# uwoseis/zephyr

Hardware: AMD Instinct MI355X
Metric: wavefields/sec (freq x source solves/s) on 1024^2 grid (higher is better)
Workload: dtype f64

## Files before the change

include/helm.h:

```cpp
#ifndef HELM_H
#define HELM_H

#include <stddef.h>

#ifdef __cplusplus
extern "C" {
#endif

typedef struct helm_op helm_op;

enum { HELM_MINIZEPHYR = 0, HELM_EURUS = 1, HELM_3D = 2  };

enum {
    HELM_BICGSTAB = 0,
    HELM_CGNR = 1,
    HELM_AUTO = 2,
    HELM_MG = 3,
    HELM_DIRECT = 4
};

enum {
    HELM_OK = 0,
    HELM_ERR_ARG = -1,
    HELM_ERR_DEVICE = -2,
// ... 140 lines not shown
    int    auto_direct;
    int    auto_mg3;
    int    prof_ext;
    int    ws_slots;
    int    pf_prio;
    int    mg3_keep;
    int    mg3_keep_levels;
    int    mg3_galerkin;
    int    mg3_depth_model;
    int    mg3_bt_f32;
    int    mg3_otf;
    int    mg3_f32;
    double mg3_omega;
    double sync_spin_ms;
    int    sync_sleep_us;
} helm_tuning;
int helm_get_tuning(helm_tuning *out);
int helm_set_tuning(const helm_tuning *t);

int helm_direct_plan(int nz, int nx, int leaf, int *out, int cap);
int helm_direct_plan_front(int nz, int nx, int leaf, int node, long long *cells, int cap);
int helm_debug_zgemm(int device, int M, int N, int K, const double *alpha, const double *A, const double *B,
                     const double *beta, double *C, int batch);
int helm_debug_inverse(int device, int n, double *A, int batch);
int helm_debug_zgemm_bench(int device, int M, int N, int K, int batch, int variant, int reps, double *ms_out);
#define HELM_ZG_TABLE 1
#define HELM_ZG_MASKS 2
#define HELM_ZG_TM64  4
int helm_debug_zgemm_choice(int M, int N, int K, int batch, int nf_div, int force_tile, int force_slab, int have_handle, int mode, int report[5]);
typedef struct helm_zgemm_ex {
// ... 42 lines not shown
```

zephyr_amd/_lib.py:

```python
import ctypes
import os
import numpy as np

_HERE = os.path.dirname(os.path.abspath(__file__))
LIB_PATH = os.path.join(_HERE, 'libhelm.so')

HELM_MINIZEPHYR, HELM_EURUS, HELM_3D = 0, 1, 2
HELM_BICGSTAB, HELM_CGNR, HELM_AUTO, HELM_MG, HELM_DIRECT = 0, 1, 2, 3, 4
HELM_RHS_NODE_MAJOR, HELM_OUT_NODE_MAJOR, HELM_NODE_MAJOR = 1, 2, 3
METHODS = {'bicgstab': HELM_BICGSTAB, 'cgnr': HELM_CGNR, 'auto': HELM_AUTO, 'mg': HELM_MG, 'direct': HELM_DIRECT}

ERRORS = {-1: 'HELM_ERR_ARG', -2: 'HELM_ERR_DEVICE', -3: 'HELM_ERR_STATE', -4: 'HELM_ERR_UNSUPPORTED', -5: 'HELM_ERR_PML'}


class HelmError(RuntimeError):
    def __init__(self, code, text):
        self.code = code
        RuntimeError.__init__(self, '%s: %s' % (ERRORS.get(code, code), text))


class SolveOpts(ctypes.Structure):
    _fields_ = [('method', ctypes.c_int), ('rtol', ctypes.c_double), ('maxit', ctypes.c_int),
                ('check_every', ctypes.c_int), ('batch', ctypes.c_int), ('flags', ctypes.c_int)]

# ... 7 lines not shown
    _fields_ = [('solve_ms', ctypes.c_double), ('apply_ms', ctypes.c_double),
                ('apply_launches', ctypes.c_longlong), ('apply_bytes', ctypes.c_double),
                ('factor_ms', ctypes.c_double), ('gemm_ms', ctypes.c_double),
                ('gemm_launches', ctypes.c_longlong), ('gemm_flops', ctypes.c_double),
                ('gemm_big_ms', ctypes.c_double), ('gemm_big_launches', ctypes.c_longlong), ('gemm_big_flops', ctypes.c_double),
                ('gemm_bytes', ctypes.c_double), ('gemm_sol_ms', ctypes.c_double)]


class Tuning(ctypes.Structure):
    _fields_ = [('nd_leaf', ctypes.c_int), ('nd_ws_gb', ctypes.c_double), ('nd_sparse_rhs', ctypes.c_int), ('nd_stable', ctypes.c_int),
                ('nd_stable_thr', ctypes.c_double), ('nd_stable_safety', ctypes.c_double), ('nd_fused_leaf', ctypes.c_int),
                ('nd_fused_leaf_min', ctypes.c_int), ('nd_gjstep', ctypes.c_int), ('nd_gjstep_min', ctypes.c_int), ('nd_overlap', ctypes.c_int),
                ('nd_xcd_map', ctypes.c_int), ('nd_plans', ctypes.c_int), ('nd_direct_out', ctypes.c_int), ('nd_many', ctypes.c_int), ('nd_leaf_idle', ctypes.c_int), ('auto_direct', ctypes.c_int),
                ('auto_mg3', ctypes.c_int), ('prof_ext', ctypes.c_int), ('ws_slots', ctypes.c_int), ('pf_prio', ctypes.c_int),
                ('mg3_keep', ctypes.c_int), ('mg3_keep_levels', ctypes.c_int), ('mg3_galerkin', ctypes.c_int), ('mg3_depth_model', ctypes.c_int),
                ('mg3_bt_f32', ctypes.c_int), ('mg3_otf', ctypes.c_int), ('mg3_f32', ctypes.c_int), ('mg3_omega', ctypes.c_double), ('sync_spin_ms', ctypes.c_double), ('sync_sleep_us', ctypes.c_int)]


class RuntimeStats(ctypes.Structure):
    _fields_ = [('dev_allocs', ctypes.c_longlong), ('dev_alloc_bytes', ctypes.c_double), ('dev_alloc_ms', ctypes.c_double),
                ('host_allocs', ctypes.c_longlong), ('host_alloc_bytes', ctypes.c_double), ('host_alloc_ms', ctypes.c_double),
                ('events_created', ctypes.c_longlong), ('streams_created', ctypes.c_longlong),
                ('first_launches', ctypes.c_longlong), ('first_launch_ms', ctypes.c_double),
                ('kernels_registered', ctypes.c_longlong), ('kernels_resolved', ctypes.c_longlong), ('warm_ms', ctypes.c_double),
                ('dev_frees', ctypes.c_longlong), ('dev_free_ms', ctypes.c_double),
                ('sync_calls', ctypes.c_longlong), ('sync_ms', ctypes.c_double), ('slow_syncs', ctypes.c_longlong), ('worst_sync_ms', ctypes.c_double)]


class ZgemmEx(ctypes.Structure):
    _fields_ = [('device', ctypes.c_int), ('M', ctypes.c_int), ('N', ctypes.c_int), ('K', ctypes.c_int), ('batch', ctypes.c_int),
                ('lda', ctypes.c_int), ('ldb', ctypes.c_int), ('ldc', ctypes.c_int),
# ... 255 lines not shown
```

zephyr_amd/csrc/nd_factor.hip:

```cpp
#include "nd_internal.hpp"
#include <map>
#include <mutex>
#include <cstring>

namespace {

__device__ __forceinline__ long long mf_off(long long off, long long slot, int nf, int kf) { return (long long)nf * off + (long long)kf * slot; }
__device__ __forceinline__ cplx *front_entry(const NdDev &n, cplx *arenaF, cplx *fac, int r, int c, int nf = 1, int kf = 0, int fac_private = 0) {
    const int nmax = n.smax + n.mmax;
    if (r < n.smax) {
        return fac + (fac_private ? n.finv_off : mf_off(n.finv_off, (long long)n.smax * nmax, nf, kf)) + (long long)r * nmax + c;
    }
    return arenaF + mf_off(n.foff, (long long)n.mmax * nmax, nf, kf) + (long long)(r - n.smax) * nmax + c;
}

__global__ __launch_bounds__(256) void k_nd_assemble(const NdDev *nodes, int first, cplx *arenaF, cplx *fac, const cplx *planes, int nz, int nx) {
    const NdDev n = nodes[first + blockIdx.y];
    const long long N = (long long)nz * nx;
    const int tot = n.s + n.m;
    for (int a = blockIdx.x * blockDim.x + threadIdx.x; a < n.smax; a += gridDim.x * blockDim.x)
        if (a >= n.s) *front_entry(n, arenaF, fac, a, a) = cmake(1.0, 0.0);
    for (int a = blockIdx.x * blockDim.x + threadIdx.x; a < tot; a += gridDim.x * blockDim.x) {
        int z, x, ca;
        nd_cell(n, a, z, x, ca);
// ... 28 lines not shown
        map[a] = nd_pos(p, nd_local(p, nz, nx, z, x, comp));
    }
    __syncthreads();
    const cplx *Sc = arenaF + c.foff + c.smax;
    const int ldc = c.smax + c.mmax;
    for (long long e0 = (long long)blockIdx.x * chunk; e0 < total; e0 += (long long)gridDim.x * chunk) {
        const long long e1 = e0 + chunk < total ? e0 + chunk : total;
        for (long long e = e0 + threadIdx.x; e < e1; e += blockDim.x) {
            const int a = (int)(e / c.m), b2 = (int)(e - (long long)a * c.m);
            cplx *dst = front_entry(p, arenaF, fac, map[a], map[b2]);
            *dst = cadd(*dst, Sc[(long long)a * ldc + b2]);
        }
    }
}

template <bool OVR>
__global__ __launch_bounds__(256) void k_nd_build_front(const NdDev *nodes, int first, cplx *arenaF, cplx *fac, NdPlanesSet pset, int nz, int nx, int rb,
                                                        int skip22, NdDev ovr, int nf, int kfix) {
    constexpr int use_ovr = OVR ? 1 : 0;
    extern __shared__ int2 finfo[];
    const int kf = kfix >= 0 ? kfix : (int)(blockIdx.y % nf);
    const cplx *planes = pset.p[kf];
    NdDev n;
    if (OVR) n = ovr; else n = nodes[first + (kfix >= 0 ? blockIdx.y : blockIdx.y / nf)];
    const int nmax = n.smax + n.mmax;
    const int r0 = blockIdx.x * rb;
    if (r0 >= nmax) return;
    const bool h0 = n.kid[0] >= 0, h1 = n.kid[1] >= 0;
    NdDev c0 = NdDev(), c1 = NdDev();
    if (h0) c0 = nodes[n.kid[0]];
    if (h1) c1 = nodes[n.kid[1]];
// ... 34 lines not shown
            if (dz >= -1 && dz <= 1 && dx >= -1 && dx <= 1) {
                if (colmode) {
                    const int dc = ((ib.x >> 24) & 0x7f) - ca;
                    if (dc >= -1 && dc <= 1) v = planes[((long long)(dc + 1) * 9 + (dz + 1) * 3 + dx + 1) * N * n.dof + (long long)ca * N + (long long)za * nx + xa];
                } else {
                    const int blk = n.dof == 2 ? 2 * ca + ((ib.y >> 28) & 1) : 0;
                    v = planes[((long long)blk * 9 + (dz + 1) * 3 + dx + 1) * N + (long long)za * nx + xa];
                }
            }
        }
        const int b0 = (colmode ? (ib.y & 0xffff) : (ib.y & 0x3fff)) - 1, b1 = (colmode ? ((ib.y >> 16) & 0xffff) : ((ib.y >> 14) & 0x3fff)) - 1;
        if (a0 >= 0 && b0 >= 0) v = cadd(v, S0[(long long)a0 * ld0 + b0]);
        if (a1 >= 0 && b1 >= 0) v = cadd(v, S1[(long long)a1 * ld1 + b1]);
        return v;
    };
    for (int r = r0 + ty; r < r1; r += 4) {
        const int2 ia = finfo[r];
        const int cend = (skip22 && r >= n.smax) ? n.smax : nmax;
        for (int c = tx; c < cend; c += 64) *front_entry(n, arenaF, fac, r, c, nf, kf, use_ovr) = value(r, c, ia, finfo[c]);
    }
}

template <int AFTER>
__global__ __launch_bounds__(256) void k_front_cond(const cplx *M0, int ld, long long stride, const NdDev *nodes, double *out, double *rows, int smax, int nf) {
    __shared__ double red[4];
    __shared__ double dsh[LUS_NMAX];
    __shared__ unsigned char lone[LUS_NMAX];
    const cplx *M = M0 + (long long)blockIdx.x * stride;
    double *w = rows + (long long)blockIdx.x * smax;
    const int n = nodes[blockIdx.x / nf].s;
    const int lane = threadIdx.x & 63, wv = threadIdx.x >> 6;
    double best = 0.0;
    for (int i = wv; i < n; i += 4) {
        double v = 0.0, off = 0.0;
// ... 311 lines not shown
    const cplx one = cmake(1, 0), mone = cmake(-1, 0);
    for (int q = 0; q < nflag; ++q) {
        const int j = h_list[1 + q];
        NdStable S;
        S.node = g.first + j; S.group = gi; S.smax = g.smax; S.mmax = g.mmax;
        S.lu = (cplx *)helm_pool_alloc(op->device, (size_t)g.smax * nmax * sizeof(cplx));
        S.f21 = (cplx *)helm_pool_alloc(op->device, (size_t)std::max(1, g.mmax) * g.smax * sizeof(cplx));
        S.piv = (int *)helm_pool_alloc(op->device, (size_t)g.smax * sizeof(int));
        f->stable.push_back(S);
        if (!S.lu || !S.f21 || !S.piv) HELM_FAIL(op, HELM_ERR_DEVICE, "direct solver: allocation for an ill-conditioned front failed");
        NdDev n = P.nodes[S.node];
        const long long foff = (long long)nf * n.foff + (long long)kf * g.mmax * nmax;
        n.finv_off = 0; n.f12_off = g.smax;
        const int rb = std::max(std::min(nmax, 4), (nmax + 2047) / 2048);
        NdPlanesSet ps; for (int q2 = 0; q2 < ND_NF_MAX; ++q2) ps.p[q2] = planes;
        HELM_LAUNCH(k_nd_build_front<true>, dim3((nmax + rb - 1) / rb, 1), dim3(256), (size_t)nmax * sizeof(int2), st, f->pd->d_nodes, 0, arenaF, S.lu, ps, P.nz, P.nx, rb,
                           0, n, nf, kf);
        cplx *F21 = arenaF + foff, *F22 = arenaF + foff + g.smax;
        HIP_TRY(op, hipMemcpy2DAsync(S.f21, (size_t)g.smax * sizeof(cplx), F21, (size_t)nmax * sizeof(cplx), (size_t)g.smax * sizeof(cplx), (size_t)g.mmax, hipMemcpyDeviceToDevice, st));
        if (g.smax <= 64) HELM_LAUNCH(k_lu_factor64, dim3(1), dim3(256), 0, st, S.lu, nmax, g.smax, S.piv);
        else HELM_LAUNCH(k_lu_factor, dim3(1), dim3(256), 0, st, S.lu, nmax, g.smax, S.piv);
        HIP_TRY(op, hipMemcpy2DAsync(work, (size_t)g.mmax * sizeof(cplx), S.lu + g.smax, (size_t)nmax * sizeof(cplx), (size_t)g.mmax * sizeof(cplx), (size_t)g.smax, hipMemcpyDeviceToDevice, st));
        HELM_LAUNCH(k_lu_solve, dim3((g.mmax + 15) / 16), dim3(256), 0, st, (const cplx *)S.lu, nmax, g.smax, (const int *)S.piv, work, g.mmax, g.mmax);
        gemm(op, g.mmax, g.mmax, g.smax, mone, S.f21, g.smax, 0, work, g.mmax, 0, one, F22, nmax, 0, 1, nullptr);
        if (getenv("HELM_ND_DEBUG") && atoi(getenv("HELM_ND_DEBUG")) >= 3) {
            auto sum2d = [&](const void *src, size_t pitch, size_t wbytes, size_t rows_) {
                std::vector<unsigned char> h(wbytes * rows_);
                hipMemcpy2D(h.data(), wbytes, src, pitch, wbytes, rows_, hipMemcpyDeviceToHost);
                unsigned long long x = 1469598103934665603ull;
                for (unsigned char c : h) { x ^= c; x *= 1099511628211ull; }
                return x;
// ... 34 lines not shown
    if (fused_leaf && g.leaf && g.cnt >= fused_leaf_min && P.dof == 1 && P.leaf <= 8 && g.smax <= 64 && g.mmax > 0 && g.mmax <= LEAF_MP) {
        const int leaf_dbg = getenv("HELM_LEAF_DBG") ? atoi(getenv("HELM_LEAF_DBG")) : 0;
        for (int k = 0; k < nf; ++k) {
            NdFactor *f = S.f[k];
            if (f->leafflag_elems < (size_t)g.cnt) {
                if (f->d_leafflag) { hipStreamSynchronize(st); helm_pool_free(op->device, f->d_leafflag, f->leafflag_elems * sizeof(int)); f->d_leafflag = nullptr; f->leafflag_elems = 0; }
                int maxcnt = g.cnt;
                for (const NdGroup &q : P.groups) if (q.leaf) maxcnt = std::max(maxcnt, q.cnt);
                f->d_leafflag = (int *)helm_pool_alloc(op->device, (size_t)maxcnt * sizeof(int));
                if (!f->d_leafflag) HELM_FAIL(op, HELM_ERR_DEVICE, "direct solver: allocation of the leaf flags failed");
                f->leafflag_elems = (size_t)maxcnt;
            }
            for (int j0 = 0; j0 < g.cnt; j0 += 65535) {
                const int nb = std::min(65535, g.cnt - j0);
                cplx *g21b = G21 + (long long)j0 * nf * g.mmax * g.smax;
                launch_leaf_factor(st, g.smax, nb, d_nodes, g.first + j0, arenaF, f0->d_fac, g21b, S.planes[k], P.nz, P.nx, f->d_leafflag + j0, leaf_dbg, nf, k);
            }
            f->flops += (double)g.cnt * 8.0 * (2.0 * LEAF_BW * g.smax * (g.smax + g.mmax) + 3.0 * g.mmax * (g.smax + g.mmax));
        }
        return HELM_OK;
    }
    bool schur_gather = false;
    const bool packs = P.dof <= 2 ? (nmax < (1 << 14) && P.nz < 65536 && P.nx < 32768) : (nmax < 65535 && P.nz < 4096 && P.nx < 4096 && P.dof < 128);
    if ((size_t)nmax * sizeof(int2) <= 64 * 1024 && packs)
        schur_gather = !g.leaf && g.mmax > 0 && P.dof == 1;
    if ((size_t)nmax * sizeof(int2) <= 64 * 1024 && packs) {
        const int want = std::max(1, 2048 / g.cnt);
        const int rb = std::max(std::min(nmax, 4), (nmax + want - 1) / want);
        NdPlanesSet ps; for (int k = 0; k < ND_NF_MAX; ++k) ps.p[k] = S.planes[k < nf ? k : 0];
        const int chunk = 65535 / nf;
        for (int j0 = 0; j0 < g.cnt; j0 += chunk) {
            const int nb = std::min(chunk, g.cnt - j0);
            HELM_LAUNCH(k_nd_build_front<false>, dim3((nmax + rb - 1) / rb, nb * nf), dim3(256), (size_t)nmax * sizeof(int2), st, d_nodes, g.first + j0, arenaF, f0->d_fac, ps,
                               P.nz, P.nx, rb, schur_gather ? 1 : 0, NdDev(), nf, -1);
        }
    } else {
        if (nf != 1) HELM_FAIL(op, HELM_ERR_UNSUPPORTED, "direct solver: fronts of %d unknowns take the unfused build, which factors one frequency at a time", nmax);
        const cplx *planes = S.planes[0];
        if (fs > 0) HIP_TRY(op, hipMemsetAsync(F, 0, (size_t)g.cnt * fs * sizeof(cplx), st));
        HIP_TRY(op, hipMemsetAsync(Finv, 0, (size_t)g.cnt * s1 * sizeof(cplx), st));
        for (int j0 = 0; j0 < g.cnt; j0 += 65535) {
            const int nb = std::min(65535, g.cnt - j0);
            HELM_LAUNCH(k_nd_assemble, dim3((nmax + 255) / 256, nb), dim3(256), 0, st, d_nodes, g.first + j0, arenaF, f0->d_fac, planes, P.nz, P.nx);
        }
        if (!g.leaf) {
            const size_t shm = (size_t)(2 * nmax + 8) * sizeof(int);
            for (int slot = 0; slot < 2; ++slot)
                for (int j0 = 0; j0 < g.cnt; j0 += 65535) {
                    const int nb = std::min(65535, g.cnt - j0);
// ... 120 lines not shown
```

zephyr_amd/csrc/nd_gemm_body.hpp:

```cpp
#pragma once
#include "nd_internal.hpp"

static __device__ cplx g_zero_page[4];
template <int WM, int WN, int MT, int NT, int IDX, int KS, int XR = 0>
__device__ __forceinline__ void zgemm3_body(int M, int Nn, int K, cplx alpha, const cplx *A0, int lda, long long sa,
                                            const cplx *B0, int ldb, long long sb, cplx beta, cplx *C0, int ldc, long long sc, const GemmRows &R,
                                            cplx *lds) {
    static_assert(WM * WN == 4 && KS % 4 == 0, "four waves per workgroup, k groups of 4");
    static_assert(!XR || (WM == 1 && (IDX == 0 || IDX == 1)), "the extra row needs all four waves side by side and plain / row-table addressing");
    constexpr int TMM = 16 * MT * WM;
    constexpr int TM = TMM + (XR ? 1 : 0), TN = 16 * NT * WN;
    constexpr int FA = TMM / 16 + (XR ? 1 : 0), FB = TN / 16, KG = KS / 4;
    constexpr int NA = (FA * 16 * KS + 255) / 256, NB = (TN * KS + 255) / 256;
    constexpr int XP = 256 / TN;
    constexpr int ABUF = KG * FA * 64, BBUF = KG * FB * 64;
    cplx *As = lds, *Bs = lds + 2 * ABUF;
    __shared__ int kidx[IDX == 1 ? GB_KIDX : 1];
    __shared__ int4 kidx4[IDX == 2 ? GB_KIDX : 1];
    int bxi = blockIdx.x, byi = blockIdx.y, bzi = blockIdx.z;
    if (gridDim.x * gridDim.y > 1 && gridDim.z >= 16 && R.la == nullptr && !(IDX == 0 && R.ksplit > 1) && R.xcd_map && (gridDim.y == 1 || R.xcd_map > 1)) {
        const int nxt = gridDim.x, nt = gridDim.x * gridDim.y, nbz = gridDim.z;
        const int L = blockIdx.x + nxt * blockIdx.y + nt * blockIdx.z;
        const int full = (nbz / 8) * 8 * nt;
        int tile;
// ... 337 lines not shown
```

zephyr_amd/csrc/nd_internal.hpp:

```cpp
#pragma once
#include "helm_internal.hpp"
#include "direct.hpp"
#include <hip/hip_ext.h>
#include <algorithm>

struct GjPivotArgs { const cplx *T0; int ld; long long stride; int n, k0, nb; const cplx *Wc0, *Wr0; long long wstride; cplx *Pb0; long long pstride; int batch; };
struct GemmRows {
    const int4 *tabB = nullptr, *tabCi = nullptr, *tabCo = nullptr;
    int offB = 0, offCi = 0, offCo = 0, tab_stride = 0;
    const cplx *Bx = nullptr, *Cix = nullptr; cplx *Cox = nullptr;
    int ldx = 0;
    int z0 = 0;
    int fwd3 = 0;
    int zr0 = 0, zr1 = 0, zc0 = 0, zc1 = 0;
    int sk0 = 0, sk1 = 0;
    int ksplit = 0, kc = 0; long long pstride = 0;
    int dense = 0;
    const cplx *Bx2 = nullptr; int k2 = 0;
    int tm64 = 0;
    const GjPivotArgs *la = nullptr;
    int schur4 = 0;
    const NdDev *nodes = nullptr; int first = 0;
    const cplx *arenaS = nullptr;
    int nf = 1;
// ... 2 lines not shown
    const int *act_ro = nullptr;
    int idle_done = 0;
    int hint = 0;
    int ntc = 0;
    int xcd_map = 0;
    int child_rows = 0;
    int cj_out = 0; cplx oscale = {1.0, 0.0}; cplx *Cox2 = nullptr;
};
#define GB_KIDX 512

#define PNB 32
#define LEAF_BW 9
#define LEAF_MP 36
#define LUS_NMAX 128
#define ND_STABLE_CAP 32

extern thread_local hipEvent_t tl_ev0, tl_ev1;
extern thread_local int tl_nf_div;
struct NfDivScope { int prev; explicit NfDivScope(int nf) : prev(tl_nf_div) { tl_nf_div = nf < 1 ? 1 : nf; } ~NfDivScope() { tl_nf_div = prev; } };
#define ZG_LAUNCH(KERNEL, GRID, ...) do { HelmFirstLaunch fl_(HelmKernelReg<(KERNEL)>::slot); \
                                          if (tl_ev0) hipExtLaunchKernelGGL(KERNEL, GRID, dim3(256), 0, st, tl_ev0, tl_ev1, 0, __VA_ARGS__); \
                                          else hipLaunchKernelGGL(KERNEL, GRID, dim3(256), 0, st, __VA_ARGS__); } while (0)

inline double gemm_operand_bytes(int M, int Nn, int K, cplx beta, const GemmRows *rows = nullptr) {
    const bool rd = !(beta.x == 0.0 && beta.y == 0.0);
    if (rows && rows->fwd3) return 16.0 * ((double)M * K + (double)K * Nn + (double)rows->child_rows * Nn + (double)M * Nn + (double)K * Nn);
    if (rows && rows->schur4) return 16.0 * ((double)M * K + (double)K * Nn + 1.5 * (double)M * Nn);
    return 16.0 * ((double)M * K + (double)K * Nn + (double)M * Nn * (rd ? 2.0 : 1.0));
}
inline double gemm_sol_ms(double flops, double bytes) { return 1e3 * std::max(flops / 78.6e12, bytes / 8.0e12); }
// ... 105 lines not shown
    }
};

struct GemmChoice { int tile = 0, kslab = 8, xr = 0, ksplit = 0, kc = 0; };
int gemm(helm_op *op, int M, int Nn, int K, cplx alpha, const cplx *A, int lda, long long sa, const cplx *B, int ldb, long long sb,
         cplx beta, cplx *C, int ldc, long long sc, int batch, const GemmRows *rows = nullptr, GemmChoice *made = nullptr);
extern int g_gemm_tile;
extern int g_gemm_slab;
extern int g_gemm_xcd;
bool gemm_sep_bwd_small(helm_op *op, int smax, int mmax, int nrhs, const cplx *Finv, const cplx *F12, int lda, long long sa, int batch, const GemmRows &rows);
void invert(helm_op *op, cplx *M, int ld, long long stride, int n, int batch, cplx *W, long long ws, int align = 1, int base = 0);
extern int g_recurse_min;
void launch_zgemm3_la(hipStream_t st, bool latency_tile, int nb, int M, int Nn, int K, cplx alpha, const cplx *A, int lda, long long sa, const cplx *B, int ldb, long long sb,
                      cplx beta, cplx *C, int ldc, long long sc, const GemmRows &R, const GjPivotArgs &pv);
void launch_leaf_factor(hipStream_t st, int smax, int nb, const NdDev *d_nodes, int first, cplx *arenaF, cplx *fac, cplx *g21b, const cplx *planes, int nz, int nx, int *flags, int dbg,
                        int nf = 1, int kf = 0);
struct FacSet { int nf = 1; NdFactor *f[ND_NF_MAX] = {nullptr, nullptr, nullptr, nullptr}; const cplx *planes[ND_NF_MAX] = {nullptr, nullptr, nullptr, nullptr}; double rtol[ND_NF_MAX] = {0, 0, 0, 0}; };
int factor_prologue(helm_op *op, int block, NdFactor *f, const cplx *planes_in, const cplx **planes);
int factor_group(helm_op *op, NdFactor *f, size_t gi, cplx *arenaF, cplx *work, const cplx *planes);
bool merged_group(const NdPlan &P, const NdGroup &g);
void launch_lu_solve(hipStream_t st, const cplx *LU, int ld, int n, const int *piv, cplx *B, int ldb, int ncols);
void launch_transpose(hipStream_t st, const cplx *in, long long rows, long long cols, cplx *out, int swap, int conj);
```

zephyr_amd/csrc/nd_leaf.hip:

```cpp
#include "nd_internal.hpp"

namespace {

#define LEAF_NB 19
#define LEAF_NBR 28
struct LeafTabs {
    int idx[LEAF_MP][3];
    cplx f12[LEAF_MP][3];
    cplx f21[LEAF_MP][3];
};
template <int SP>
__device__ __forceinline__ void leaf_load(const NdDev &n, const cplx *planes, int nz, int nx, cplx *band, float *rowmax, int *brow, LeafTabs &T, int tid, int nthreads) {
    const long long N = (long long)nz * nx;
    const int w = n.x1 - n.x0, h = n.z1 - n.z0;
    for (int e = tid; e < SP * LEAF_NB; e += nthreads) band[e] = (e % LEAF_NB == LEAF_BW && e / LEAF_NB >= n.s) ? cmake(1.0, 0.0) : cmake(0.0, 0.0);
    for (int a = tid; a < SP; a += nthreads) {
        int br = -1;
        if (a < n.s) {
            const int lz = a / w, lx = a % w;
            if (lz == 0 || lz == h - 1 || lx == 0 || lx == w - 1) {
                int cnt = 0;
                for (int q = 0; q < a; ++q) { const int qz = q / w, qx = q % w; if (qz == 0 || qz == h - 1 || qx == 0 || qx == w - 1) cnt += 1; }
                br = cnt;
            }
        }
        brow[a] = br;
        rowmax[a] = 1.0f;
    }
    for (int e = tid; e < LEAF_MP * 3; e += nthreads) { T.idx[e / 3][e % 3] = -1; T.f12[e / 3][e % 3] = cmake(0.0, 0.0); T.f21[e / 3][e % 3] = cmake(0.0, 0.0); }
}
template <int SP>
__device__ __forceinline__ void leaf_fill(const NdDev &n, const cplx *planes, int nz, int nx, cplx *band, float *rowmax, LeafTabs &T, int tid, int nthreads) {
    const long long N = (long long)nz * nx;
    const int w = n.x1 - n.x0;
    for (int a = tid; a < n.s; a += nthreads) {
        const int z = n.z0 + a / w, x = n.x0 + a % w;
        float mx = 0.f;
        #pragma unroll
        for (int k = 0; k < 9; ++k) {
            const int z2 = z + k / 3 - 1, x2 = x + k % 3 - 1;
            if (z2 < n.z0 || z2 >= n.z1 || x2 < n.x0 || x2 >= n.x1) continue;
            const cplx v = planes[(long long)k * N + (long long)z * nx + x];
            const int b = (z2 - n.z0) * w + (x2 - n.x0);
// ... 6 lines not shown
        int zr, xr;
        nd_cell(n, n.s + r, zr, xr);
        int t = 0;
        for (int k = 0; k < 9; ++k) {
            const int z2 = zr + k / 3 - 1, x2 = xr + k % 3 - 1;
            if (z2 < n.z0 || z2 >= n.z1 || x2 < n.x0 || x2 >= n.x1 || t >= 3) continue;
            const int a = (z2 - n.z0) * w + (x2 - n.x0);
            T.idx[r][t] = a;
            T.f21[r][t] = planes[(long long)k * N + (long long)zr * nx + xr];
            T.f12[r][t] = planes[(long long)(8 - k) * N + (long long)z2 * nx + x2];
            t += 1;
        }
    }
}

template <int SP>
__global__ __launch_bounds__(128, 4) void k_leaf_factor(const NdDev *nodes, int first, cplx *arenaF, cplx *fac, cplx *g21base, const cplx *planes, int nz, int nx, int *flags, int dbg,
                                                        int nf, int kf) {
    __shared__ cplx band[SP * LEAF_NB];
    __shared__ LeafTabs T;
    __shared__ float rowmax[SP];
    __shared__ int brow[SP];
    __shared__ int bad;
    const NdDev n = nodes[first + blockIdx.x];
    const int tid = threadIdx.x;
    const int smax = n.smax, mmax = n.mmax, nmax = smax + mmax;
    if (tid == 0) bad = 0;
    leaf_load<SP>(n, planes, nz, nx, band, rowmax, brow, T, tid, 128);
    __syncthreads();
    leaf_fill<SP>(n, planes, nz, nx, band, rowmax, T, tid, 128);
    __syncthreads();
    if (tid < 64 && !(dbg & 1)) {
        int mybad = 0;
        for (int k = 0; k < SP; ++k) {
            const cplx p = band[k * LEAF_NB + LEAF_BW];
            const double pm = fmax(fabs(p.x), fabs(p.y));
            if (!(pm >= 0.01 * (double)rowmax[k])) mybad = 1;
            const cplx pi = crecip(p);
            for (int e = tid; e < LEAF_BW * LEAF_BW; e += 64) {
                const int di = e / LEAF_BW + 1, dj = e % LEAF_BW + 1;
                const int i = k + di, j = k + dj;
                if (i < SP && j < SP) {
                    const cplx l = cmul(band[i * LEAF_NB + LEAF_BW - di], pi);
// ... 58 lines not shown
                if (i - AHEAD >= 0) yq[i - AHEAD] = (stored && i - AHEAD < smax) ? Fcol[(long long)(i - AHEAD) * nmax] : LEAF_RHS(i - AHEAD);
                cplx nxt = cur;
                if (i > 0) nxt = band[(i - 1) * LEAF_NB + lb];
                cplx acc = yq[i];
                #pragma unroll
                for (int d = 1; d <= LEAF_BW; ++d)
                    if (i + d < SP) { const cplx u = bcast(cur, LEAF_BW + d); acc.x = fma(u.y, xw[i + d].y, fma(-u.x, xw[i + d].x, acc.x)); acc.y = fma(-u.y, xw[i + d].x, fma(-u.x, xw[i + d].y, acc.y)); }
                acc = cmul(acc, bcast(cur, LEAF_BW));
                xw[i] = acc;
                if (stored && i < smax) Fcol[(long long)i * nmax] = acc;
                cur = nxt;
            }
        }
    }
    __syncthreads();
    if (active && !(dbg & 4)) {
        cplx *G21 = g21base + ((long long)blockIdx.x * nf + kf) * mmax * smax;
        cplx *S = arenaF + (long long)nf * n.foff + (long long)kf * mmax * nmax + smax;
        for (int r = 0; r < mmax; ++r) {
            cplx acc = cmake(0.0, 0.0);
            if (r < n.m && stored) {
                #pragma unroll
                for (int t = 0; t < 3; ++t) {
                    const int a = T.idx[r][t];
                    if (a >= 0) cfma(acc, T.f21[r][t], Fcol[(long long)a * nmax]);
                }
            }
            if (c < SP) { if (c < smax) G21[(long long)r * smax + c] = acc; }
            else S[(long long)r * nmax + (c - SP)] = acc;
        }
    }
}

// ... 61 lines not shown
                        const int q = T.idx[r][t];
                        if (q < 0) continue;
                        cplx gqb = cmake(0.0, 0.0);
                        for (int u = 0; u < 3; ++u) { const int q2 = T.idx[b][u]; if (q2 >= 0) cfma(gqb, a[q][q2], cneg(T.f12[b][u])); }
                        cfma(v, T.f21[r][t], gqb);
                    }
            }
        }
        if (cc < smax) G21[(long long)r * smax + cc] = v; else S[(long long)r * nmax + (cc - smax)] = v;
    }
}

}

void launch_leaf_factor(hipStream_t st, int smax, int nb, const NdDev *d_nodes, int first, cplx *arenaF, cplx *fac, cplx *g21b, const cplx *planes, int nz, int nx, int *flags, int dbg,
                        int nf, int kf) {
    if (smax <= 49) HELM_LAUNCH(k_leaf_factor<49>, dim3(nb), dim3(128), 0, st, d_nodes, first, arenaF, fac, g21b, planes, nz, nx, flags, dbg, nf, kf);
    else HELM_LAUNCH(k_leaf_factor<64>, dim3(nb), dim3(128), 0, st, d_nodes, first, arenaF, fac, g21b, planes, nz, nx, flags, dbg, nf, kf);
    HELM_LAUNCH(k_leaf_factor_pivoted, dim3(nb), dim3(256), 0, st, d_nodes, first, arenaF, fac, g21b, planes, nz, nx, (const int *)flags, nf, kf);
}
```

zephyr_amd/csrc/runtime.hip:

```cpp
#include "helm_internal.hpp"
#include <chrono>
#include <atomic>
#include <unistd.h>
#include <time.h>
#include <mutex>
#include <thread>
#include <map>
#include <cstring>
#include <algorithm>

namespace {
struct KernelRec { const void *fn; const char *pretty; std::atomic<bool> launched{false}; };
struct KernelRegistry {
    std::mutex mu;
    std::vector<KernelRec *> recs;
    std::atomic<KernelRec *> fast[2048];
    std::atomic<int> n{0};
};
KernelRegistry &kreg() { static KernelRegistry *r = new KernelRegistry(); return *r; }
struct RuntimeCounters {
    std::atomic<long long> dev_frees{0}, dev_free_us{0}, sync_calls{0}, sync_us{0}, slow_syncs{0}, worst_sync_us{0};
    std::atomic<long long> dev_allocs{0}, dev_alloc_bytes{0}, dev_alloc_us{0}, host_allocs{0}, host_alloc_bytes{0}, host_alloc_us{0},
                           events{0}, streams{0}, first_launches{0}, first_launch_us{0}, resolved{0}, warm_us{0};
};
// ... 161 lines not shown
int helm_env_int(const char *name, int d) { const char *v = getenv(name); return v ? atoi(v) : d; }
namespace {
std::mutex g_tune_mu;
bool g_tune_set = false;
helm_tuning g_tune_user;
double tune_d(const char *name, double d) { const char *v = getenv(name); return v ? atof(v) : d; }
}
static void tuning_clamp(helm_tuning &t) {
    t.nd_leaf = std::max(2, t.nd_leaf);
    if (!(t.nd_ws_gb > 0)) t.nd_ws_gb = 32.0;
    t.nd_stable_safety = std::max(1.0, t.nd_stable_safety);
    if (!(t.nd_stable_thr >= 0)) t.nd_stable_thr = 0.0;
    t.nd_fused_leaf_min = std::max(1, t.nd_fused_leaf_min);
    t.nd_gjstep_min = std::max(64, t.nd_gjstep_min);
    t.nd_plans = std::max(1, t.nd_plans);
    t.ws_slots = std::min(4, std::max(1, t.ws_slots));
    t.pf_prio = t.pf_prio > 0 ? 1 : (t.pf_prio < 0 ? -1 : 0);
    if (!(t.mg3_omega > 0) || t.mg3_omega > 2.0) t.mg3_omega = 0.9;
    if (!(t.sync_spin_ms >= 0)) t.sync_spin_ms = 0.0;
    t.sync_spin_ms = std::min(t.sync_spin_ms, 60000.0);
    t.sync_sleep_us = std::min(100000, std::max(0, t.sync_sleep_us));
}
static helm_tuning tuning_from_env() {
    helm_tuning t;
    t.nd_leaf = helm_env_int("HELM_ND_LEAF", 8);
    t.nd_ws_gb = tune_d("HELM_ND_WS_GB", 32.0);
    t.nd_sparse_rhs = helm_env_int("HELM_ND_SPARSE_RHS", 1);
    t.nd_stable = helm_env_int("HELM_ND_STABLE", 1);
    t.nd_stable_thr = tune_d("HELM_ND_STABLE_THR", 0.0);
    t.nd_stable_safety = tune_d("HELM_ND_STABLE_SAFETY", 8.0);
    t.nd_fused_leaf = helm_env_int("HELM_ND_FUSEDLEAF", 1);
    t.nd_fused_leaf_min = helm_env_int("HELM_ND_FUSEDLEAF_MIN", 2048);
    t.nd_gjstep = helm_env_int("HELM_ND_GJSTEP", 1);
    t.nd_gjstep_min = helm_env_int("HELM_ND_GJSTEP_MIN", 128);
    t.nd_overlap = helm_env_int("HELM_ND_OVERLAP_NM", 1);
    t.nd_xcd_map = helm_env_int("HELM_ND_XCDMAP", 2);
    t.nd_plans = helm_env_int("HELM_ND_PLANS", 6);
    t.nd_direct_out = helm_env_int("HELM_ND_DIRECT_OUT", 1);
    t.nd_leaf_idle = helm_env_int("HELM_ND_LEAF_IDLE", 1);
    t.nd_many = helm_env_int("HELM_ND_MANY", 1);
    t.auto_direct = helm_env_int("HELM_AUTO_DIRECT", 1);
    t.auto_mg3 = helm_env_int("HELM_AUTO_MG3", 1);
    t.prof_ext = helm_env_int("HELM_PROF_EXT", 1);
    t.ws_slots = helm_env_int("HELM_WS_SLOTS", 3);
    t.pf_prio = helm_env_int("HELM_PF_PRIO", 1);
    t.mg3_keep = helm_env_int("HELM_MG3_KEEP", 1);
    t.mg3_keep_levels = helm_env_int("HELM_MG3_KEEP_LEVELS", -1);
    t.mg3_galerkin = helm_env_int("HELM_MG3_GALERKIN", 1);
    t.mg3_depth_model = helm_env_int("HELM_MG3_DEPTH_MODEL", 1);
    t.mg3_bt_f32 = helm_env_int("HELM_MG3_BT_F32", 1);
    t.mg3_otf = helm_env_int("HELM_MG3_OTF", 1);
    t.mg3_f32 = helm_env_int("HELM_MG3_F32", 1);
    t.mg3_omega = tune_d("HELM_MG3_OMEGA", 0.9);
    t.sync_spin_ms = tune_d("HELM_SYNC_SPIN_MS", 0.0);
    t.sync_sleep_us = helm_env_int("HELM_SYNC_SLEEP_US", 0);
// ... 555 lines not shown
```

Before: 15870.

## Batch independent gathers in front build and leaf G21/Schur writeback

Adds a tunable nd_gather mode, on by default, under which the fused front-build kernel handles several entries per thread. Each thread first computes all addresses, using a zero page for padded entries, then issues the loads together before combining and storing, so gather latency can overlap. The leaf factor kernel gets a similar batched path for the G21/Schur writeback, plus __restrict__ qualifiers. It also drops the unused O(n^2) boundary-row count from leaf_load. The risks are higher register pressure and a larger code footprint.

```diff
diff --git a/include/helm.h b/include/helm.h
--- a/include/helm.h
+++ b/include/helm.h
@@ -178,6 +178,7 @@
     double mg3_omega;
     double sync_spin_ms;
     int    sync_sleep_us;
+    int    nd_gather;
 } helm_tuning;
 int helm_get_tuning(helm_tuning *out);
 int helm_set_tuning(const helm_tuning *t);
diff --git a/zephyr_amd/_lib.py b/zephyr_amd/_lib.py
--- a/zephyr_amd/_lib.py
+++ b/zephyr_amd/_lib.py
@@ -45,7 +45,8 @@
                 ('nd_xcd_map', ctypes.c_int), ('nd_plans', ctypes.c_int), ('nd_direct_out', ctypes.c_int), ('nd_many', ctypes.c_int), ('nd_leaf_idle', ctypes.c_int), ('auto_direct', ctypes.c_int),
                 ('auto_mg3', ctypes.c_int), ('prof_ext', ctypes.c_int), ('ws_slots', ctypes.c_int), ('pf_prio', ctypes.c_int),
                 ('mg3_keep', ctypes.c_int), ('mg3_keep_levels', ctypes.c_int), ('mg3_galerkin', ctypes.c_int), ('mg3_depth_model', ctypes.c_int),
-                ('mg3_bt_f32', ctypes.c_int), ('mg3_otf', ctypes.c_int), ('mg3_f32', ctypes.c_int), ('mg3_omega', ctypes.c_double), ('sync_spin_ms', ctypes.c_double), ('sync_sleep_us', ctypes.c_int)]
+                ('mg3_bt_f32', ctypes.c_int), ('mg3_otf', ctypes.c_int), ('mg3_f32', ctypes.c_int), ('mg3_omega', ctypes.c_double), ('sync_spin_ms', ctypes.c_double), ('sync_sleep_us', ctypes.c_int),
+                ('nd_gather', ctypes.c_int)]
 
 
 class RuntimeStats(ctypes.Structure):
diff --git a/zephyr_amd/csrc/nd_factor.hip b/zephyr_amd/csrc/nd_factor.hip
--- a/zephyr_amd/csrc/nd_factor.hip
+++ b/zephyr_amd/csrc/nd_factor.hip
@@ -66,7 +66,7 @@
     }
 }
 
-template <bool OVR>
+template <bool OVR, int R>
 __global__ __launch_bounds__(256) void k_nd_build_front(const NdDev *nodes, int first, cplx *arenaF, cplx *fac, NdPlanesSet pset, int nz, int nx, int rb,
                                                         int skip22, NdDev ovr, int nf, int kfix) {
     constexpr int use_ovr = OVR ? 1 : 0;
@@ -131,10 +131,65 @@
         if (a1 >= 0 && b1 >= 0) v = cadd(v, S1[(long long)a1 * ld1 + b1]);
         return v;
     };
-    for (int r = r0 + ty; r < r1; r += 4) {
-        const int2 ia = finfo[r];
-        const int cend = (skip22 && r >= n.smax) ? n.smax : nmax;
-        for (int c = tx; c < cend; c += 64) *front_entry(n, arenaF, fac, r, c, nf, kf, use_ovr) = value(r, c, ia, finfo[c]);
+    if (R == 0) {
+        for (int r = r0 + ty; r < r1; r += 4) {
+            const int2 ia = finfo[r];
+            const int cend = (skip22 && r >= n.smax) ? n.smax : nmax;
+            for (int c = tx; c < cend; c += 64) *front_entry(n, arenaF, fac, r, c, nf, kf, use_ovr) = value(r, c, ia, finfo[c]);
+        }
+        return;
+    }
+    constexpr int RR = R > 0 ? R : 1;
+    const int smax_ = n.smax;
+    for (int region = 0; region < 2; ++region) {
+        const int ra = region == 0 ? r0 : max(r0, smax_), re = region == 0 ? min(r1, smax_) : r1;
+        const int W = (region == 1 && skip22) ? smax_ : nmax;
+        if (ra >= re || W <= 0) continue;
+        int lwlog = 6;
+        if (W < 64) { lwlog = 0; while ((1 << lwlog) < W) lwlog += 1; }
+        const int G = 64 >> lwlog, sub = tx >> lwlog, cl = tx & ((1 << lwlog) - 1);
+        const int nch = (W + 63) >> 6;
+        int rw = ra + ty * G, ch = 0;
+        while (rw < re) {
+            int rr[RR], cc[RR];
+            bool on[RR], pad[RR], h0q[RR], h1q[RR], diag[RR];
+            const cplx *ps[RR], *p0[RR], *p1[RR];
+            #pragma unroll
+            for (int j = 0; j < RR; ++j) {
+                const int r = rw + sub, c = (ch << 6) + cl;
+                rr[j] = r; cc[j] = c;
+                on[j] = rw < re && r < re && c < W;
+                if (++ch == nch) { ch = 0; rw += 4 * G; }
+                const int2 ia = finfo[on[j] ? r : 0], ib = finfo[on[j] ? c : 0];
+                pad[j] = !on[j] || ia.x < 0 || ib.x < 0;
+                diag[j] = r == c && r < smax_;
+                const int za = colmode ? (ia.x & 0xfff) : (ia.x & 0xffff), xa = colmode ? ((ia.x >> 12) & 0xfff) : (ia.x >> 16);
+                const int ca = colmode ? ((ia.x >> 24) & 0x7f) : ((ia.y >> 28) & 1);
+                const int zb = colmode ? (ib.x & 0xfff) : (ib.x & 0xffff), xb = colmode ? ((ib.x >> 12) & 0xfff) : (ib.x >> 16);
+                const int cb = colmode ? ((ib.x >> 24) & 0x7f) : ((ib.y >> 28) & 1);
+                const int a0 = (colmode ? (ia.y & 0xffff) : (ia.y & 0x3fff)) - 1, a1 = (colmode ? ((ia.y >> 16) & 0xffff) : ((ia.y >> 14) & 0x3fff)) - 1;
+                const int b0 = (colmode ? (ib.y & 0xffff) : (ib.y & 0x3fff)) - 1, b1 = (colmode ? ((ib.y >> 16) & 0xffff) : ((ib.y >> 14) & 0x3fff)) - 1;
+                const int dz = zb - za, dx = xb - xa, dc = colmode ? cb - ca : 0;
+                const bool st = !pad[j] && (r < smax_ || c < smax_) && dz >= -1 && dz <= 1 && dx >= -1 && dx <= 1 && dc >= -1 && dc <= 1;
+                const long long plane = colmode ? ((long long)(dc + 1) * 9 + (dz + 1) * 3 + dx + 1) * n.dof
+                                                : (long long)(n.dof == 2 ? 2 * ca + cb : 0) * 9 + (dz + 1) * 3 + dx + 1;
+                ps[j] = st ? planes + plane * N + (colmode ? (long long)ca * N : 0) + (long long)za * nx + xa : g_zero_page;
+                h0q[j] = !pad[j] && a0 >= 0 && b0 >= 0;
+                h1q[j] = !pad[j] && a1 >= 0 && b1 >= 0;
+                p0[j] = h0q[j] ? S0 + (long long)a0 * ld0 + b0 : g_zero_page;
+                p1[j] = h1q[j] ? S1 + (long long)a1 * ld1 + b1 : g_zero_page;
+            }
+            cplx xs[RR], x0[RR], x1[RR];
+            #pragma unroll
+            for (int j = 0; j < RR; ++j) { xs[j] = *ps[j]; x0[j] = *p0[j]; x1[j] = *p1[j]; }
+            #pragma unroll
+            for (int j = 0; j < RR; ++j) {
+                cplx v = pad[j] ? cmake(diag[j] ? 1.0 : 0.0, 0.0) : xs[j];
+                v = h0q[j] ? cadd(v, x0[j]) : v;
+                v = h1q[j] ? cadd(v, x1[j]) : v;
+                if (on[j]) *front_entry(n, arenaF, fac, rr[j], cc[j], nf, kf, use_ovr) = v;
+            }
+        }
     }
 }
 
@@ -476,7 +531,7 @@
         n.finv_off = 0; n.f12_off = g.smax;
         const int rb = std::max(std::min(nmax, 4), (nmax + 2047) / 2048);
         NdPlanesSet ps; for (int q2 = 0; q2 < ND_NF_MAX; ++q2) ps.p[q2] = planes;
-        HELM_LAUNCH(k_nd_build_front<true>, dim3((nmax + rb - 1) / rb, 1), dim3(256), (size_t)nmax * sizeof(int2), st, f->pd->d_nodes, 0, arenaF, S.lu, ps, P.nz, P.nx, rb,
+        HELM_LAUNCH((k_nd_build_front<true, 0>), dim3((nmax + rb - 1) / rb, 1), dim3(256), (size_t)nmax * sizeof(int2), st, f->pd->d_nodes, 0, arenaF, S.lu, ps, P.nz, P.nx, rb,
                            0, n, nf, kf);
         cplx *F21 = arenaF + foff, *F22 = arenaF + foff + g.smax;
         HIP_TRY(op, hipMemcpy2DAsync(S.f21, (size_t)g.smax * sizeof(cplx), F21, (size_t)nmax * sizeof(cplx), (size_t)g.smax * sizeof(cplx), (size_t)g.mmax, hipMemcpyDeviceToDevice, st));
@@ -541,7 +596,7 @@
             for (int j0 = 0; j0 < g.cnt; j0 += 65535) {
                 const int nb = std::min(65535, g.cnt - j0);
                 cplx *g21b = G21 + (long long)j0 * nf * g.mmax * g.smax;
-                launch_leaf_factor(st, g.smax, nb, d_nodes, g.first + j0, arenaF, f0->d_fac, g21b, S.planes[k], P.nz, P.nx, f->d_leafflag + j0, leaf_dbg, nf, k);
+                launch_leaf_factor(st, g.smax, nb, d_nodes, g.first + j0, arenaF, f0->d_fac, g21b, S.planes[k], P.nz, P.nx, f->d_leafflag + j0, leaf_dbg, nf, k, tune.nd_gather);
             }
             f->flops += (double)g.cnt * 8.0 * (2.0 * LEAF_BW * g.smax * (g.smax + g.mmax) + 3.0 * g.mmax * (g.smax + g.mmax));
         }
@@ -558,8 +613,15 @@
         const int chunk = 65535 / nf;
         for (int j0 = 0; j0 < g.cnt; j0 += chunk) {
             const int nb = std::min(chunk, g.cnt - j0);
-            HELM_LAUNCH(k_nd_build_front<false>, dim3((nmax + rb - 1) / rb, nb * nf), dim3(256), (size_t)nmax * sizeof(int2), st, d_nodes, g.first + j0, arenaF, f0->d_fac, ps,
-                               P.nz, P.nx, rb, schur_gather ? 1 : 0, NdDev(), nf, -1);
+            if (tune.nd_gather == 0)
+                HELM_LAUNCH((k_nd_build_front<false, 0>), dim3((nmax + rb - 1) / rb, nb * nf), dim3(256), (size_t)nmax * sizeof(int2), st, d_nodes, g.first + j0, arenaF, f0->d_fac, ps,
+                                   P.nz, P.nx, rb, schur_gather ? 1 : 0, NdDev(), nf, -1);
+            else if (tune.nd_gather == 2)
+                HELM_LAUNCH((k_nd_build_front<false, 2>), dim3((nmax + rb - 1) / rb, nb * nf), dim3(256), (size_t)nmax * sizeof(int2), st, d_nodes, g.first + j0, arenaF, f0->d_fac, ps,
+                                   P.nz, P.nx, rb, schur_gather ? 1 : 0, NdDev(), nf, -1);
+            else
+                HELM_LAUNCH((k_nd_build_front<false, 4>), dim3((nmax + rb - 1) / rb, nb * nf), dim3(256), (size_t)nmax * sizeof(int2), st, d_nodes, g.first + j0, arenaF, f0->d_fac, ps,
+                                   P.nz, P.nx, rb, schur_gather ? 1 : 0, NdDev(), nf, -1);
         }
     } else {
         if (nf != 1) HELM_FAIL(op, HELM_ERR_UNSUPPORTED, "direct solver: fronts of %d unknowns take the unfused build, which factors one frequency at a time", nmax);
diff --git a/zephyr_amd/csrc/nd_gemm_body.hpp b/zephyr_amd/csrc/nd_gemm_body.hpp
--- a/zephyr_amd/csrc/nd_gemm_body.hpp
+++ b/zephyr_amd/csrc/nd_gemm_body.hpp
@@ -1,7 +1,6 @@
 #pragma once
 #include "nd_internal.hpp"
 
-static __device__ cplx g_zero_page[4];
 template <int WM, int WN, int MT, int NT, int IDX, int KS, int XR = 0>
 __device__ __forceinline__ void zgemm3_body(int M, int Nn, int K, cplx alpha, const cplx *A0, int lda, long long sa,
                                             const cplx *B0, int ldb, long long sb, cplx beta, cplx *C0, int ldc, long long sc, const GemmRows &R,
diff --git a/zephyr_amd/csrc/nd_internal.hpp b/zephyr_amd/csrc/nd_internal.hpp
--- a/zephyr_amd/csrc/nd_internal.hpp
+++ b/zephyr_amd/csrc/nd_internal.hpp
@@ -40,6 +40,8 @@
 #define LEAF_MP 36
 #define LUS_NMAX 128
 #define ND_STABLE_CAP 32
+
+static __device__ cplx g_zero_page[4];
 
 extern thread_local hipEvent_t tl_ev0, tl_ev1;
 extern thread_local int tl_nf_div;
@@ -175,7 +177,7 @@
 void launch_zgemm3_la(hipStream_t st, bool latency_tile, int nb, int M, int Nn, int K, cplx alpha, const cplx *A, int lda, long long sa, const cplx *B, int ldb, long long sb,
                       cplx beta, cplx *C, int ldc, long long sc, const GemmRows &R, const GjPivotArgs &pv);
 void launch_leaf_factor(hipStream_t st, int smax, int nb, const NdDev *d_nodes, int first, cplx *arenaF, cplx *fac, cplx *g21b, const cplx *planes, int nz, int nx, int *flags, int dbg,
-                        int nf = 1, int kf = 0);
+                        int nf = 1, int kf = 0, int gather = 1);
 struct FacSet { int nf = 1; NdFactor *f[ND_NF_MAX] = {nullptr, nullptr, nullptr, nullptr}; const cplx *planes[ND_NF_MAX] = {nullptr, nullptr, nullptr, nullptr}; double rtol[ND_NF_MAX] = {0, 0, 0, 0}; };
 int factor_prologue(helm_op *op, int block, NdFactor *f, const cplx *planes_in, const cplx **planes);
 int factor_group(helm_op *op, NdFactor *f, size_t gi, cplx *arenaF, cplx *work, const cplx *planes);
diff --git a/zephyr_amd/csrc/nd_leaf.hip b/zephyr_amd/csrc/nd_leaf.hip
--- a/zephyr_amd/csrc/nd_leaf.hip
+++ b/zephyr_amd/csrc/nd_leaf.hip
@@ -3,30 +3,15 @@
 namespace {
 
 #define LEAF_NB 19
-#define LEAF_NBR 28
 struct LeafTabs {
     int idx[LEAF_MP][3];
     cplx f12[LEAF_MP][3];
     cplx f21[LEAF_MP][3];
 };
 template <int SP>
-__device__ __forceinline__ void leaf_load(const NdDev &n, const cplx *planes, int nz, int nx, cplx *band, float *rowmax, int *brow, LeafTabs &T, int tid, int nthreads) {
-    const long long N = (long long)nz * nx;
-    const int w = n.x1 - n.x0, h = n.z1 - n.z0;
+__device__ __forceinline__ void leaf_load(const NdDev &n, cplx *band, float *rowmax, LeafTabs &T, int tid, int nthreads) {
     for (int e = tid; e < SP * LEAF_NB; e += nthreads) band[e] = (e % LEAF_NB == LEAF_BW && e / LEAF_NB >= n.s) ? cmake(1.0, 0.0) : cmake(0.0, 0.0);
-    for (int a = tid; a < SP; a += nthreads) {
-        int br = -1;
-        if (a < n.s) {
-            const int lz = a / w, lx = a % w;
-            if (lz == 0 || lz == h - 1 || lx == 0 || lx == w - 1) {
-                int cnt = 0;
-                for (int q = 0; q < a; ++q) { const int qz = q / w, qx = q % w; if (qz == 0 || qz == h - 1 || qx == 0 || qx == w - 1) cnt += 1; }
-                br = cnt;
-            }
-        }
-        brow[a] = br;
-        rowmax[a] = 1.0f;
-    }
+    for (int a = tid; a < SP; a += nthreads) rowmax[a] = 1.0f;
     for (int e = tid; e < LEAF_MP * 3; e += nthreads) { T.idx[e / 3][e % 3] = -1; T.f12[e / 3][e % 3] = cmake(0.0, 0.0); T.f21[e / 3][e % 3] = cmake(0.0, 0.0); }
 }
 template <int SP>
@@ -63,19 +48,19 @@
     }
 }
 
+#define LEAF_RB 4
 template <int SP>
-__global__ __launch_bounds__(128, 4) void k_leaf_factor(const NdDev *nodes, int first, cplx *arenaF, cplx *fac, cplx *g21base, const cplx *planes, int nz, int nx, int *flags, int dbg,
-                                                        int nf, int kf) {
+__global__ __launch_bounds__(128, 4) void k_leaf_factor(const NdDev *nodes, int first, cplx *__restrict__ arenaF, cplx *__restrict__ fac, cplx *__restrict__ g21base, const cplx *planes,
+                                                        int nz, int nx, int *flags, int dbg, int nf, int kf, int gather) {
     __shared__ cplx band[SP * LEAF_NB];
     __shared__ LeafTabs T;
     __shared__ float rowmax[SP];
-    __shared__ int brow[SP];
     __shared__ int bad;
     const NdDev n = nodes[first + blockIdx.x];
     const int tid = threadIdx.x;
     const int smax = n.smax, mmax = n.mmax, nmax = smax + mmax;
     if (tid == 0) bad = 0;
-    leaf_load<SP>(n, planes, nz, nx, band, rowmax, brow, T, tid, 128);
+    leaf_load<SP>(n, band, rowmax, T, tid, 128);
     __syncthreads();
     leaf_fill<SP>(n, planes, nz, nx, band, rowmax, T, tid, 128);
     __syncthreads();
@@ -164,9 +149,36 @@
         }
     }
     __syncthreads();
-    if (active && !(dbg & 4)) {
-        cplx *G21 = g21base + ((long long)blockIdx.x * nf + kf) * mmax * smax;
-        cplx *S = arenaF + (long long)nf * n.foff + (long long)kf * mmax * nmax + smax;
+    cplx *G21 = g21base + ((long long)blockIdx.x * nf + kf) * mmax * smax;
+    cplx *S = arenaF + (long long)nf * n.foff + (long long)kf * mmax * nmax + smax;
+    if (active && gather && !(dbg & 4)) {
+        for (int rq = 0; rq < mmax; rq += LEAF_RB) {
+            cplx x[LEAF_RB][3], f[LEAF_RB][3];
+            bool ok[LEAF_RB][3];
+            #pragma unroll
+            for (int j = 0; j < LEAF_RB; ++j) {
+                const int r = rq + j < LEAF_MP ? rq + j : LEAF_MP - 1;
+                #pragma unroll
+                for (int t = 0; t < 3; ++t) {
+                    const int a = T.idx[r][t];
+                    ok[j][t] = rq + j < n.m && stored && a >= 0;
+                    f[j][t] = T.f21[r][t];
+                    x[j][t] = *(ok[j][t] ? Fcol + (long long)a * nmax : g_zero_page);
+                }
+            }
+            #pragma unroll
+            for (int j = 0; j < LEAF_RB; ++j) {
+                const int r = rq + j;
+                cplx acc = cmake(0.0, 0.0);
+                #pragma unroll
+                for (int t = 0; t < 3; ++t) { cplx w = acc; cfma(w, f[j][t], x[j][t]); acc.x = ok[j][t] ? w.x : acc.x; acc.y = ok[j][t] ? w.y : acc.y; }
+                if (r < mmax) {
+                    if (c < SP) { if (c < smax) G21[(long long)r * smax + c] = acc; }
+                    else S[(long long)r * nmax + (c - SP)] = acc;
+                }
+            }
+        }
+    } else if (active && !(dbg & 4)) {
         for (int r = 0; r < mmax; ++r) {
             cplx acc = cmake(0.0, 0.0);
             if (r < n.m && stored) {
@@ -258,8 +270,8 @@
 }
 
 void launch_leaf_factor(hipStream_t st, int smax, int nb, const NdDev *d_nodes, int first, cplx *arenaF, cplx *fac, cplx *g21b, const cplx *planes, int nz, int nx, int *flags, int dbg,
-                        int nf, int kf) {
-    if (smax <= 49) HELM_LAUNCH(k_leaf_factor<49>, dim3(nb), dim3(128), 0, st, d_nodes, first, arenaF, fac, g21b, planes, nz, nx, flags, dbg, nf, kf);
-    else HELM_LAUNCH(k_leaf_factor<64>, dim3(nb), dim3(128), 0, st, d_nodes, first, arenaF, fac, g21b, planes, nz, nx, flags, dbg, nf, kf);
+                        int nf, int kf, int gather) {
+    if (smax <= 49) HELM_LAUNCH(k_leaf_factor<49>, dim3(nb), dim3(128), 0, st, d_nodes, first, arenaF, fac, g21b, planes, nz, nx, flags, dbg, nf, kf, gather);
+    else HELM_LAUNCH(k_leaf_factor<64>, dim3(nb), dim3(128), 0, st, d_nodes, first, arenaF, fac, g21b, planes, nz, nx, flags, dbg, nf, kf, gather);
     HELM_LAUNCH(k_leaf_factor_pivoted, dim3(nb), dim3(256), 0, st, d_nodes, first, arenaF, fac, g21b, planes, nz, nx, (const int *)flags, nf, kf);
 }
diff --git a/zephyr_amd/csrc/runtime.hip b/zephyr_amd/csrc/runtime.hip
--- a/zephyr_amd/csrc/runtime.hip
+++ b/zephyr_amd/csrc/runtime.hip
@@ -199,6 +199,7 @@
     t.nd_fused_leaf_min = std::max(1, t.nd_fused_leaf_min);
     t.nd_gjstep_min = std::max(64, t.nd_gjstep_min);
     t.nd_plans = std::max(1, t.nd_plans);
+    if (t.nd_gather != 0 && t.nd_gather != 2 && t.nd_gather != 4) t.nd_gather = 1;
     t.ws_slots = std::min(4, std::max(1, t.ws_slots));
     t.pf_prio = t.pf_prio > 0 ? 1 : (t.pf_prio < 0 ? -1 : 0);
     if (!(t.mg3_omega > 0) || t.mg3_omega > 2.0) t.mg3_omega = 0.9;
@@ -224,6 +225,7 @@
     t.nd_direct_out = helm_env_int("HELM_ND_DIRECT_OUT", 1);
     t.nd_leaf_idle = helm_env_int("HELM_ND_LEAF_IDLE", 1);
     t.nd_many = helm_env_int("HELM_ND_MANY", 1);
+    t.nd_gather = helm_env_int("HELM_ND_GATHER", 1);
     t.auto_direct = helm_env_int("HELM_AUTO_DIRECT", 1);
     t.auto_mg3 = helm_env_int("HELM_AUTO_MG3", 1);
     t.prof_ext = helm_env_int("HELM_PROF_EXT", 1);
```

After: 15970, median of 6. About the same (+0.6%).
